# TrondVQ/UncertaintyQuantification-SleepApnea-1DCNN

Measured on AMD Instinct MI355X. Metric: 30s-windows/sec for MCD T=50 & DE M=8 inference at 1/2/4/8 MI355X, higher is better.
Workload: dtype fp32; 1 GPU; global_batch=16384, seq_len=60, parallelism=dp1, mcd_passes=50, de_members=8, bn_mode_mcd=batch

## Files before the change

### uncertaintyquantification_sleepapnea_1dcnn_amd/csrc/x3_layers.hip

```cpp
#include "common.h"
#include "f16x3.h"
#include "x3_api.h"
#include "x3_dense_map.h"

namespace apneauq {
namespace x3 {

constexpr int kStagers = 4;
constexpr int kL = 60, kSR = 64, kHalo = 4;
__host__ __device__ constexpr int row_bytes(int ck) { return 4 * ck + 32; }
__device__ __forceinline__ int sample_prescale(unsigned rmax_bits, const float* amax) {
  return prescale_exp(__builtin_fmaf(amax[0], __uint_as_float(rmax_bits), amax[1]));
}

__host__ __device__ constexpr int lds_rows(int S) { return kHalo + S * kSR + kHalo; }
__host__ __device__ constexpr int buf_bytes(int S, int ck) { return lds_rows(S) * row_bytes(ck); }
__host__ __device__ constexpr int tab_rows(int S, int ks) { return kSR * S + (ks - 1); }
__host__ __device__ constexpr int lds_bytes(int S, int cout, int ck, int ks, bool dense_rows = false) {
  return 2 * (dense_rows ? dense::lds_rows(kSR * S) * row_bytes(ck) : buf_bytes(S, ck)) + 2 * cout * 8 + 2 * S * 4 +
         (dense_rows ? 2 * kSR * S * 4 + 2 * tab_rows(S, ks) * 8 : 0);
}

template <typename T>
__device__ __forceinline__ T gld(const void* p) {
  return *(const __attribute__((address_space(1))) T*)(p);
}

__device__ __forceinline__ int opaque_tid() {
  int t = threadIdx.x;
  asm volatile("" : "+v"(t));
  return t;
}

__device__ __forceinline__ void lds_barrier() {
  __builtin_amdgcn_fence(__ATOMIC_RELEASE, "workgroup", "local");
  __builtin_amdgcn_s_barrier();
  __builtin_amdgcn_fence(__ATOMIC_ACQUIRE, "workgroup", "local");
}

template <int NW, int WPC>
constexpr int waves_per_eu() { return NW * WPC > 8 ? (NW * WPC + 3) / 4 : NW * WPC <= 4 ? 1 : 2; }
constexpr int loaders(int lw) { return lw > 0 ? lw : 0; }
template <int CIN, int COUT, int KS, int S, int WM, int WN, bool LAST, int LW, int CK, int WPC, bool PS, bool DENSE = false>
__global__ __launch_bounds__((WM * WN + loaders(LW)) * 64, (waves_per_eu<WM * WN + loaders(LW), WPC>())) void layer_kernel(
    const LayerArgs A) {
  extern __shared__ __attribute__((aligned(16))) char smem[];
  constexpr int NWM = WM * WN, NW = NWM + loaders(LW), kThreads = NW * 64;
  constexpr int kCK = CK, kRowB = row_bytes(CK), NQ = CK / 32, kQ = CK / 4;
  constexpr int PAD = (KS - 1) / 2, kRows = kSR * S;
  static_assert(!DENSE || (!PS && !LAST), "dense rows: batch-moment blocks 2..5 only");
  constexpr int kS = S, kBufB = DENSE ? dense::lds_rows(kRows) * kRowB : buf_bytes(S, CK);
  constexpr int kValidRows = DENSE ? kRows : S * kL, kUnits = kValidRows * kQ;
  constexpr int SW = LW > 0 ? LW : LW < 0 ? (-LW < NW ? -LW : NW) : (kStagers < NW ? kStagers : NW);
  constexpr int kSBase = LW > 0 ? NWM * 64 : 0;
  constexpr int kST = SW * 64;
  constexpr int kMainU = (kUnits + kST - 1) / kST, kNU = kMainU + (DENSE ? 1 : 0);
  constexpr int kEdgeWaves = (2 * PAD * kQ + 63) / 64;
  static_assert(!DENSE || (kUnits % kST == 0 && kEdgeWaves <= SW), "dense rows: whole staging steps per tile");
  static_assert(kST % kQ == 0 && (CK == 32 || CK == 64), "a staging thread keeps one channel quad");
  constexpr int NCH = CIN / kCK, NCTA = COUT / 16, NCT = NCTA / WN, NRT = 4 * S / WM;
  constexpr int NSTEP = NCH * NQ * KS;
  constexpr int RG = NCT >= 4                        ? 1
                     : (NCT >= 3 && NCT * NRT > 16)    ? 1
                     : NCT == 1                        ? 4
                                                       : 2;
  constexpr bool BDB = NCT * NRT <= 24 && RG < 4;
  static_assert(NRT % RG == 0, "row-tile groups");
  constexpr long long FRAG_STEP = (long long)NCTA * 128;
  static_assert(CIN % kCK == 0 && COUT % 16 == 0, "channel tiling");
  static_assert(NCTA % WN == 0 && (4 * S) % WM == 0, "wave tiling");
  static_assert(NRT % 4 == 0, "whole 64-row sample slots per wave row (epilogue keys, block 6 sums)");
  double* st = reinterpret_cast<double*>(smem + 2 * kBufB);
  float* wsc = reinterpret_cast<float*>(smem + 2 * kBufB + 2 * COUT * 8);
  constexpr int kTabRows = tab_rows(S, KS);
  static_assert(!DENSE || CIN / CK >= 2, "row tables: a tile's tables are written one chunk of the same workgroup ahead");
  unsigned* ektab = reinterpret_cast<unsigned*>(smem + 2 * kBufB + 2 * COUT * 8 + 2 * S * 4);
  uint2* stab = reinterpret_cast<uint2*>(smem + 2 * kBufB + 2 * COUT * 8 + 2 * S * 4 + 2 * kRows * 4);

  const int tid = threadIdx.x, lane = tid & 63;
  const int wave = __builtin_amdgcn_readfirstlane(tid >> 6);
  const int wn = wave % WN, wm = (wave / WN) % WM;
  const int ct0 = wn * NCT, rt0 = wm * NRT;
  const int m = lane & 15, h = lane >> 4;
  APNEAUQ_DASSERT(blockDim.x == kThreads);

  const int wg = xcd_order(blockIdx.x, gridDim.x);
  const int tpg = DENSE ? (int)dense::tiles(A.n_win, kRows) : (A.n_win + S - 1) / S;
  const int total_tiles = tpg * A.groups;
  const int t_begin = (int)((long long)wg * total_tiles / gridDim.x);
  const int t_end = (int)((long long)(wg + 1) * total_tiles / gridDim.x);
  if (t_begin >= t_end) return;
  const int slot = wg % kStatSlots;

  const bool loader = LW > 0 && wave >= NWM;
  const bool stager = LW > 0 ? loader : wave < SW;
  const bool edge_wave = DENSE && wave >= kSBase / 64 && wave - kSBase / 64 < kEdgeWaves;
  auto unit_row = [&](int u, int tid, int& rel) -> bool {
    const int r = tid / kQ;
    if (u < kMainU) {
      rel = r + (kST / kQ) * u;
      return true;
    }
    rel = r < PAD ? r - PAD : kRows - PAD + r;
    return edge_wave && r < 2 * PAD;
  };
  struct Stage {
    f32x4 v[kNU];
    f32x4 a, b;
  };
  Stage s0;
  const bool hash_in = A.thr_in != 0u && !A.sign_in;
  const bool sign_in = A.thr_in != 0u && A.sign_in;
  const bool prescale = PS && A.smax_in != nullptr;
  int key_tile = -1;
  unsigned skeys[kS];
  unsigned skey_tile = 0u;
  static_assert(kS <= 8, "packed per-sample exponents");
  constexpr int kSP = (kS + 3) / 4;
  unsigned sa_pack[kSP];
  struct Geo {
    int g, w0, wf, off, rows_left;
  };
  auto tile_geo = [&](int tile) {
    Geo G;
    G.g = tile / tpg;
    G.w0 = (tile - G.g * tpg) * (DENSE ? kRows : kS);
    G.wf = DENSE ? G.w0 / kL : G.w0, G.off = DENSE ? G.w0 - G.wf * kL : 0;
    const long long left = (long long)(A.n_win - G.wf) * kL - G.off;
    G.rows_left = (int)(left < 1024 ? left : 1024);
    return G;
  };
  const bool mask_out = DENSE && A.sign_out && A.thr_out != 0u;
  auto write_tables = [&](int tile) {
    if constexpr (DENSE) {
      const int tid = opaque_tid() - kSBase;
      const Geo G = tile_geo(tile);
      const unsigned ikey = stream_key(A.seed, A.layer - 1, A.pass_base + G.g);
      const unsigned okey = stream_key(A.seed, A.layer, A.pass_base + G.g);
#pragma unroll
      for (int i0 = 0; i0 < kTabRows; i0 += kST) {
        const int i = i0 + tid, rel = i - PAD;
        if (i < kTabRows) {
          const unsigned d = dense::row_desc(rel, G.off, kRows, PAD, G.rows_left);
          const unsigned win = A.window_offset + G.wf + dense::desc_slot(d);
          const int t = dense::desc_step(d);
          stab[(tile & 1) * kTabRows + i] = uint2{d, hash_in ? dense::mask_word(sample_key(ikey, win), t) : 0u};
          if (mask_out && rel >= 0 && rel < kRows) ektab[(tile & 1) * kRows + rel] = dense::mask_word(sample_key(okey, win), t);
        }
      }
    }
  };
  auto load_chunk = [&](int tile, int c, Stage& R) {
    const int tid = opaque_tid() - kSBase, q = tid % kQ;
    const Geo G = tile_geo(tile);
    const float* af = A.aff_in + (long long)G.g * A.aff_gstride + c * kCK + 4 * q;
    R.a = gld<f32x4>(af);
    R.b = gld<f32x4>(af + CIN);
    if constexpr (DENSE) {
      const long long row0 = (A.in_shared ? 0ll : (long long)G.g * A.n_win * kL) + G.w0;
      const float* in = A.in + row0 * CIN + c * kCK + 4 * q;
#pragma unroll
      for (int u = 0; u < kNU; ++u) {
        int rel;
        bool have = unit_row(u, tid, rel);
        if (u >= kMainU) have = have && dense::staged(G.off + rel, G.off, kRows, PAD);
        R.v[u] = f32x4{-0.f, -0.f, -0.f, -0.f};
        if (have && rel < G.rows_left) R.v[u] = gld<f32x4>(in + rel * CIN);
      }
    } else {
#pragma unroll
      for (int u = 0; u < kNU; ++u) {
        const int ri = tid / kQ + (kST / kQ) * u;
        R.v[u] = f32x4{-0.f, -0.f, -0.f, -0.f};
        if (ri < kValidRows) {
          const int s = ri / kL, t = ri - s * kL, w = G.w0 + s;
          if (w < A.n_win) {
            const long long si = A.in_shared ? w : (long long)G.g * A.n_win + w;
            R.v[u] = gld<f32x4>(A.in + (si * kL + t) * CIN + c * kCK + 4 * q);
          }
        }
      }
    }
  };
  auto store_chunk = [&](int tile, int c, char* buf, const Stage& R) {
    const int tid = opaque_tid() - kSBase, q = tid % kQ;
    const int g = tile / tpg;
    const int w0 = (tile - g * tpg) * (DENSE ? kRows : kS);
    if (DENSE && c == NCH - 1 && tile + 1 < t_end) write_tables(tile + 1);
    if (tile != key_tile) {
      const unsigned skey = stream_key(A.seed, A.layer - 1, A.pass_base + g);
      skey_tile = skey;
      const float* am = A.amax_in + (A.aff_gstride ? 2 * g : 0);
      float ws0 = A.wscale[A.p_gstride ? g : 0];
      if (A.gscale_in != nullptr) ws0 *= A.gscale_in[A.aff_gstride ? g : 0];
#pragma unroll
      for (int i = 0; i < kSP; ++i) sa_pack[i] = 0u;
      if (DENSE && tid == 0) wsc[(tile & 1) * kS] = ws0;
#pragma unroll
      for (int s = 0; s < (DENSE ? 0 : kS); ++s) {
        skeys[s] = sample_key(skey, A.window_offset + w0 + s);
        int sa = 0;
        if (prescale && w0 + s < A.n_win) {
          const long long si = A.in_shared ? w0 + s : (long long)g * A.n_win + w0 + s;
          sa = sample_prescale(A.smax_in[si], am);
          sa_pack[s >> 2] |= ((unsigned)sa & 0xFFu) << (8 * (s & 3));
        }
        if (tid == s) wsc[(tile & 1) * kS + s] = ldexpf(ws0, -sa);
      }
      key_tile = tile;
    }
    const uint2* tab = stab + (tile & 1) * kTabRows + PAD;
#pragma unroll
    for (int u = 0; u < kNU; ++u) {
      int s, lrow;
      bool valid;
      unsigned kt = 0u;
      if constexpr (DENSE) {
        int rel;
        if (!unit_row(u, tid, rel)) continue;
        const uint2 e = tab[rel];
        if (e.x == 0u) continue;
        s = dense::desc_slot(e.x), lrow = dense::desc_lds_row(e.x), valid = dense::desc_valid(e.x), kt = e.y;
      } else {
        const int ri = tid / kQ + (kST / kQ) * u;
        if (ri >= kValidRows) continue;
        s = ri / kL;
        const int t = ri - s * kL;
        lrow = kHalo + s * kSR + t, valid = w0 + s < A.n_win;
        if (hash_in) {
          unsigned k;
          if constexpr (!PS) {
            k = sample_key(skey_tile, A.window_offset + w0 + s);
          } else {
            k = skeys[0];
#pragma unroll
            for (int j = 1; j < kS; ++j) k = s == j ? skeys[j] : k;
          }
          kt = dense::mask_word(k, t);
        }
      }
      const f32x4 v = R.v[u];
      bool keep[4];
      if (hash_in) {
        const unsigned cp = (unsigned)(c * kCK + 4 * q) >> 1;
        const unsigned b01 = mix32(kt ^ cp), b23 = mix32(kt ^ (cp + 1u));
        keep[0] = (b01 & 0xFFFFu) >= A.thr_in;
        keep[1] = (b01 >> 16) >= A.thr_in;
        keep[2] = (b23 & 0xFFFFu) >= A.thr_in;
        keep[3] = (b23 >> 16) >= A.thr_in;
      } else if (sign_in) {
#pragma unroll
        for (int i = 0; i < 4; ++i) keep[i] = !__builtin_signbit(v[i]);
      } else {
#pragma unroll
        for (int i = 0; i < 4; ++i) keep[i] = true;
      }
      int sa = 0;
      if (prescale) {
        unsigned sp = sa_pack[0];
#pragma unroll
        for (int i = 1; i < kSP; ++i) sp = (s >> 2) == i ? sa_pack[i] : sp;
        sa = __builtin_amdgcn_sbfe((int)sp, 8 * (s & 3), 8);
      }
      float a[4];
#pragma unroll
      for (int i = 0; i < 4; ++i) a[i] = (valid && keep[i]) ? ldexpf(__builtin_fmaf(v[i], R.a[i], R.b[i]), sa) : 0.f;
      uint2 hi, lo;
      split2(a[0], a[1], hi.x, lo.x);
      split2(a[2], a[3], hi.y, lo.y);
      char* row = buf + lrow * kRowB + 8 * q;
      *reinterpret_cast<uint2*>(row) = hi;
      *reinterpret_cast<uint2*>(row + 2 * kCK) = lo;
    }
  };

  f32x4 acc[NCT][NRT];
#pragma unroll
  for (int ct = 0; ct < NCT; ++ct)
#pragma unroll
    for (int rt = 0; rt < NRT; ++rt) acc[ct][rt] = f32x4{0.f, 0.f, 0.f, 0.f};
  auto wbase = [&](int tile) -> const gf16x8* {
    const int g = tile / tpg;
    return (const gf16x8*)(A.wfrag) + (long long)g * A.w_gstride + ct0 * 128 + lane;
  };
  f16x8 ah[NCT], al[NCT];
  auto load_a = [&](const gf16x8* p, f16x8 (&xh)[NCT], f16x8 (&xl)[NCT]) {
#pragma unroll
    for (int ct = 0; ct < NCT; ++ct) {
      xh[ct] = p[ct * 128];
      xl[ct] = p[ct * 128 + 64];
    }
  };

  const int bofs = ((rt0 * 16 + m + kHalo - PAD) * kRowB) + 16 * h;

  auto compute_chunk = [&](int c, int off, const char* buf, const gf16x8* wcur, const gf16x8* wnxt, auto&& hook) {
    const char* bp[DENSE ? NRT : 1];
    if constexpr (DENSE) {
#pragma unroll
      for (int rt = 0; rt < NRT; ++rt)
        bp[rt] = buf + bofs + (off + (dense::kSlot - kL) * ((off + (rt0 + rt) * 16 + m) / kL)) * kRowB;
    }
#pragma unroll
    for (int kk = 0; kk < NQ * KS; ++kk) {
      const int q2 = kk / KS, j = kk - q2 * KS;
      const char* bb = buf + bofs + q2 * 64;
      const int s = c * NQ * KS + kk;
      const gf16x8* np = (s + 1 < NSTEP) ? wcur + (long long)(s + 1) * FRAG_STEP : wnxt;
      f16x8 nh[NCT], nl[NCT];
      load_a(np, nh, nl);
      __builtin_amdgcn_sched_barrier(0);
      auto ldb = [&](int rt, f16x8& h_, f16x8& l_) {
        const char* br = DENSE ? bp[rt] + q2 * 64 : bb;
        h_ = *reinterpret_cast<const f16x8*>(br + (rt * 16 + j) * kRowB);
        l_ = *reinterpret_cast<const f16x8*>(br + (rt * 16 + j) * kRowB + 2 * kCK);
      };
      f16x8 bh[RG], bl[RG];
#pragma unroll
      for (int r = 0; r < RG; ++r) ldb(r, bh[r], bl[r]);
#pragma unroll
      for (int rg = 0; rg < NRT; rg += RG) {
        f16x8 bh2[RG], bl2[RG];
#pragma unroll
        for (int r = 0; r < RG; ++r) {
          bh2[r] = bh[r];
          bl2[r] = bl[r];
          if (BDB && rg + RG < NRT) ldb(rg + RG + r, bh2[r], bl2[r]);
          if (!BDB) ldb(rg + r, bh[r], bl[r]);
        }
        __builtin_amdgcn_sched_barrier(0);
#pragma unroll
        for (int r = 0; r < RG; ++r)
#pragma unroll
          for (int ct = 0; ct < NCT; ++ct) acc[ct][rg + r] = mfma(ah[ct], bh[r], acc[ct][rg + r]);
#pragma unroll
        for (int r = 0; r < RG; ++r)
#pragma unroll
          for (int ct = 0; ct < NCT; ++ct) acc[ct][rg + r] = mfma(al[ct], bh[r], acc[ct][rg + r]);
#pragma unroll
        for (int r = 0; r < RG; ++r)
#pragma unroll
          for (int ct = 0; ct < NCT; ++ct) acc[ct][rg + r] = mfma(ah[ct], bl[r], acc[ct][rg + r]);
#pragma unroll
        for (int r = 0; r < RG; ++r) {
          bh[r] = bh2[r];
          bl[r] = bl2[r];
        }
      }
#pragma unroll
      for (int ct = 0; ct < NCT; ++ct) {
        ah[ct] = nh[ct];
        al[ct] = nl[ct];
      }
      __builtin_amdgcn_sched_barrier(0);
      if (kk == (NQ * KS) / 2) hook();
    }
  };

  auto epilogue = [&](int tile) {
    const int lane = opaque_tid() & 63, m = lane & 15, h = lane >> 4;
    const int g = tile / tpg;
    const int w0 = (tile - g * tpg) * (DENSE ? kRows : kS);
    float wsq[NRT / 4];
#pragma unroll
    for (int q = 0; q < NRT / 4; ++q) wsq[q] = wsc[(tile & 1) * kS + (DENSE ? 0 : (rt0 >> 2) + q)];
    const bool track = PS && !LAST && A.smax_out != nullptr;
    float mxs[NRT / 4];
#pragma unroll
    for (int q = 0; q < NRT / 4; ++q) mxs[q] = 0.f;
    const float* bias = A.bias + (long long)g * A.p_gstride;
    const bool drop = (LAST || A.sign_out) && A.thr_out != 0u;
    constexpr int NKEY = DENSE ? 1 : NRT / 4;
    unsigned skeys[NKEY];
    if (!DENSE && drop) {
      const unsigned skey = stream_key(A.seed, A.layer, A.pass_base + g);
#pragma unroll
      for (int q = 0; q < NKEY; ++q) skeys[q] = sample_key(skey, A.window_offset + w0 + (rt0 >> 2) + q);
    }
    const long long left = (long long)A.n_win * kL - w0;
    const int rows_left = DENSE ? (int)(left < kRows ? left : kRows) : 0;
#pragma unroll
    for (int ct = 0; ct < NCT; ++ct) {
      const int co0 = (ct0 + ct) * 16 + 4 * h;
      const f32x4 b4 = gld<f32x4>(bias + co0);
      f32x4 s1 = {0.f, 0.f, 0.f, 0.f}, s2 = s1, k1 = s1, k0 = s1;
      int mo = m;
      if constexpr (DENSE) asm volatile("" : "+v"(mo));
      const int rel0 = rt0 * 16 + mo;
      const unsigned* ek = ektab + (tile & 1) * kRows + rel0;
      float* orow = DENSE ? A.out + (((long long)g * A.n_win * kL + w0 + rel0) * COUT + co0) : nullptr;
#pragma unroll
      for (int rt = 0; rt < NRT; ++rt) {
        int t = 0, w = 0;
        bool valid;
        if constexpr (DENSE) {
          valid = rel0 + rt * 16 < rows_left;
        } else {
          const int s = (rt0 + rt) >> 2;
          t = (((rt0 + rt) & 3) << 4) + m, w = w0 + s, valid = t < kL && w < A.n_win;
        }
        f32x4 r;
#pragma unroll
        for (int e = 0; e < 4; ++e) r[e] = fmaxf(__builtin_fmaf(acc[ct][rt][e], wsq[rt >> 2], b4[e]), 0.f);
        acc[ct][rt] = f32x4{0.f, 0.f, 0.f, 0.f};
        bool keep[4] = {true, true, true, true};
        if (drop) {
          unsigned b01, b23;
          if constexpr (DENSE) {
            const unsigned kt = ek[rt * 16];
            b01 = mix32(kt ^ ((unsigned)co0 >> 1)), b23 = mix32(kt ^ (((unsigned)co0 >> 1) + 1u));
          } else {
            b01 = dropout_bits2(skeys[rt >> 2], t, co0), b23 = dropout_bits2(skeys[rt >> 2], t, co0 + 2);
          }
          keep[0] = (b01 & 0xFFFFu) >= A.thr_out;
          keep[1] = (b01 >> 16) >= A.thr_out;
          keep[2] = (b23 & 0xFFFFu) >= A.thr_out;
          keep[3] = (b23 >> 16) >= A.thr_out;
        }
        if (valid) {
#pragma unroll
          for (int e = 0; e < 4; ++e) {
            s1[e] += r[e];
            s2[e] = __builtin_fmaf(r[e], r[e], s2[e]);
            if (!LAST) mxs[rt >> 2] = fmaxf(mxs[rt >> 2], r[e]);
            if constexpr (LAST) {
              k1[e] += keep[e] ? r[e] : 0.f;
              k0[e] += keep[e] ? 1.f : 0.f;
            }
          }
          if constexpr (!LAST) {
            const long long sample = (long long)g * A.n_win + w;
            f32x4 o = r;
            if (drop) {
#pragma unroll
              for (int e = 0; e < 4; ++e) o[e] = keep[e] ? r[e] : __builtin_copysignf(r[e], -1.f);
            }
            if constexpr (DENSE)
              *reinterpret_cast<f32x4*>(orow + rt * 16 * COUT) = o;
            else
              *reinterpret_cast<f32x4*>(A.out + (sample * kL + t) * COUT + co0) = o;
          }
        }
        if constexpr (LAST) {
          if ((rt & 3) == 3) {
#pragma unroll
            for (int e = 0; e < 4; ++e) {
              k1[e] = group16_sum(k1[e]);
              k0[e] = group16_sum(k0[e]);
            }
            const int wl = w0 + (rt0 + rt) / 4;
            if (m == 0 && wl < A.n_win) {
              float* o = A.out + ((long long)g * A.n_win + wl) * (2 * COUT);
              *reinterpret_cast<f32x4*>(o + co0) = k1;
              *reinterpret_cast<f32x4*>(o + COUT + co0) = k0;
            }
            k1 = f32x4{0.f, 0.f, 0.f, 0.f};
            k0 = k1;
          }
        }
      }
      if (A.stats != nullptr) {
#pragma unroll
        for (int e = 0; e < 4; ++e) {
          const float a = group16_sum(s1[e]), b = group16_sum(s2[e]);
          if (m == 0) {
            atomicAdd(&st[co0 + e], (double)a);
            atomicAdd(&st[COUT + co0 + e], (double)b);
          }
        }
      }
    }
    if (track) {
#pragma unroll
      for (int q = 0; q < NRT / 4; ++q) {
        const float mq = wave_max(mxs[q]);
        const int w = w0 + (rt0 >> 2) + q;
        if (lane == 0 && w < A.n_win) atomicMax(A.smax_out + (long long)g * A.n_win + w, __float_as_uint(mq));
      }
    }
  };

  auto flush_stats = [&](int g) {
    __syncthreads();
    if (A.stats != nullptr) {
      double* dst = A.stats + ((long long)g * kStatSlots + slot) * 2 * COUT;
      for (int i = DENSE ? opaque_tid() : tid; i < 2 * COUT; i += kThreads) {
        atomicAdd(dst + i, st[i]);
        st[i] = 0.0;
      }
    }
    __syncthreads();
  };

  for (int i = tid; i < 2 * kBufB / 16; i += kThreads) reinterpret_cast<f32x4*>(smem)[i] = f32x4{0.f, 0.f, 0.f, 0.f};
  for (int i = tid; i < 2 * COUT; i += kThreads) st[i] = 0.0;
  if (DENSE && stager) write_tables(t_begin);
  __syncthreads();
  const int total = (t_end - t_begin) * NCH;
  auto chunk_tile = [&](int it) { return t_begin + it / NCH; };
  auto tile_off = [&](int tile) { return DENSE ? (int)((long long)(tile % tpg) * kRows % kL) : 0; };
  int g_cur = t_begin / tpg;
  if constexpr (LW > 0) {
    if (loader) {
      if (stager) {
        load_chunk(t_begin, 0, s0);
        store_chunk(t_begin, 0, smem, s0);
      }
      lds_barrier();
      if (stager && total > 1) load_chunk(chunk_tile(1), 1 % NCH, s0);
#pragma unroll 1
      for (int it = 0; it < total; ++it) {
        const int tile = chunk_tile(it), c = it - (tile - t_begin) * NCH;
        if (c == 0) {
          const int g = tile / tpg;
          if (g != g_cur) {
            flush_stats(g_cur);
            g_cur = g;
          }
        }
        if (stager && it + 1 < total) store_chunk(chunk_tile(it + 1), (it + 1) % NCH, smem + ((it + 1) & 1) * kBufB, s0);
        lds_barrier();
        if (stager && it + 2 < total) load_chunk(chunk_tile(it + 2), (it + 2) % NCH, s0);
      }
      flush_stats(g_cur);
      return;
    }
    lds_barrier();
    load_a(wbase(t_begin), ah, al);
#pragma unroll 1
    for (int it = 0; it < total; ++it) {
      const int tile = chunk_tile(it), c = it - (tile - t_begin) * NCH;
      if (c == 0) {
        const int g = tile / tpg;
        if (g != g_cur) {
          flush_stats(g_cur);
          g_cur = g;
        }
      }
      const gf16x8* wcur = wbase(tile);
      const gf16x8* wnxt = wbase(tile + 1 < t_end ? tile + 1 : tile);
      compute_chunk(c, tile_off(tile), smem + (it & 1) * kBufB, wcur, wnxt, []() {});
      if (c == NCH - 1) epilogue(tile);
      lds_barrier();
    }
    flush_stats(g_cur);
    return;
  }
  if (stager) {
    load_chunk(t_begin, 0, s0);
    store_chunk(t_begin, 0, smem, s0);
  }
  lds_barrier();
  if (stager && total > 1) load_chunk(chunk_tile(1), 1 % NCH, s0);
  load_a(wbase(t_begin), ah, al);
#pragma unroll 1
  for (int it = 0; it < total; ++it) {
    const int tile = chunk_tile(it), c = it - (tile - t_begin) * NCH;
    if (c == 0) {
      const int g = tile / tpg;
      if (g != g_cur) {
        flush_stats(g_cur);
        g_cur = g;
      }
    }
    const gf16x8* wcur = wbase(tile);
    const gf16x8* wnxt = wbase(tile + 1 < t_end ? tile + 1 : tile);
    char* buf = smem + (it & 1) * kBufB;
    char* nbuf = smem + ((it + 1) & 1) * kBufB;
    compute_chunk(c, tile_off(tile), buf, wcur, wnxt, [&]() {
      if (stager && it + 1 < total) store_chunk(chunk_tile(it + 1), (it + 1) % NCH, nbuf, s0);
    });
    if (c == NCH - 1) epilogue(tile);
    lds_barrier();
    if (stager && it + 2 < total) load_chunk(chunk_tile(it + 2), (it + 2) % NCH, s0);
  }
  flush_stats(g_cur);
}

__global__ __launch_bounds__(256) void l1_kernel(const L1Args A) {
  __shared__ float xs[kL1Win][kL + 6][4];
  __shared__ float red[2][2][128];
  __shared__ unsigned wmax[kL1Win];
  const int g = blockIdx.x / A.blocks_per_group;
  const int w0 = (blockIdx.x - g * A.blocks_per_group) * kL1Win;
  const int tid = threadIdx.x, c = tid & 127, half = tid >> 7;
  for (int i = tid; i < kL1Win * (kL + 6) * 4; i += 256) {
    const int s = i / ((kL + 6) * 4), r = (i / 4) % (kL + 6), ci = i & 3;
    const int t = r - 3, w = w0 + s;
    xs[s][r][ci] = (t >= 0 && t < kL && w < A.n_win) ? A.x[((long long)w * kL + t) * 4 + ci] : 0.f;
  }
  float wr[7][4];
#pragma unroll
  for (int j = 0; j < 7; ++j)
#pragma unroll
    for (int ci = 0; ci < 4; ++ci) wr[j][ci] = A.w[(((long long)g * 7 + j) * 4 + ci) * 128 + c];
  const float bc = A.b[g * 128 + c];
  if (tid < kL1Win) wmax[tid] = 0u;
  __syncthreads();
  float s1 = 0.f, s2 = 0.f;
  for (int s = 0; s < kL1Win; ++s) {
    const int w = w0 + s;
    if (w >= A.n_win) break;
    float* o = A.out + (((long long)g * A.n_win + w) * kL) * 128 + c;
    float mx = 0.f;
    for (int t = half * 30; t < half * 30 + 30; ++t) {
      float v = bc;
#pragma unroll
      for (int j = 0; j < 7; ++j)
#pragma unroll
        for (int ci = 0; ci < 4; ++ci) v = __builtin_fmaf(xs[s][t + j][ci], wr[j][ci], v);
      v = fmaxf(v, 0.f);
      o[t * 128] = v;
      s1 += v;
      s2 = __builtin_fmaf(v, v, s2);
      mx = fmaxf(mx, v);
    }
    if (A.smax != nullptr) {
      mx = wave_max(mx);
      if ((tid & 63) == 0) atomicMax(&wmax[s], __float_as_uint(mx));
    }
  }
  if (A.stats != nullptr || A.smax != nullptr) {
    red[half][0][c] = s1;
    red[half][1][c] = s2;
    __syncthreads();
    if (A.stats != nullptr && tid < 128) {
      double* dst = A.stats + ((long long)g * kStatSlots + (blockIdx.x % kStatSlots)) * 2 * 128;
      atomicAdd(dst + c, (double)red[0][0][c] + (double)red[1][0][c]);
      atomicAdd(dst + 128 + c, (double)red[0][1][c] + (double)red[1][1][c]);
    }
    if (A.smax != nullptr && tid < kL1Win && w0 + tid < A.n_win) A.smax[(long long)g * A.n_win + w0 + tid] = wmax[tid];
  }
}

__device__ __forceinline__ void aff_moments(const AffArgs& A, int g, int c, float& mean, float& var) {
  const double* p = A.stats + (long long)g * kStatSlots * 2 * A.C + c;
  double a = 0.0, b = 0.0;
#pragma unroll
  for (int s = 0; s < kStatSlots; ++s) {
    a += p[s * 2 * A.C];
    b += p[s * 2 * A.C + A.C];
  }
  const double mu = a * A.inv_count;
  mean = (float)mu;
  var = (float)fmax(b * A.inv_count - mu * mu, 0.0);
}

__global__ __launch_bounds__(256) void aff_kernel(const AffArgs A) {
  __shared__ float red[2][4];
  const int tid = threadIdx.x;
  if ((int)blockIdx.x == A.groups) {
    for (int c = tid; c < A.C; c += 256)
      for (int g = 0; g < A.groups; ++g) {
        const long long po = (long long)g * A.p_gstride + c;
        float mean, var;
        aff_moments(A, g, c, mean, var);
        for (int r = 0; r < A.repeat; ++r) {
          A.mmean[po] = A.mmean[po] * A.momentum + mean * (1.f - A.momentum);
          A.mvar[po] = A.mvar[po] * A.momentum + var * (1.f - A.momentum);
        }
      }
    return;
  }
  {
    const int g = blockIdx.x;
    float ms = 0.f, mt = 0.f;
    for (int c = tid; c < A.C; c += 256) {
      const long long po = (long long)g * A.p_gstride + c;
      float mean, var;
      if (A.stats != nullptr && !A.running) {
        aff_moments(A, g, c, mean, var);
      } else {
        mean = A.mmean[po];
        var = A.mvar[po];
      }
      const float sc = A.gamma[po] / sqrtf(var + A.eps);
      const float s_ = sc * A.dsc, t_ = (A.beta[po] - mean * sc) * A.dsc;
      A.aff[((long long)g * 2) * A.C + c] = s_;
      A.aff[((long long)g * 2 + 1) * A.C + c] = t_;
      if (A.gscale != nullptr) {
        const double* p = A.stats + (long long)g * kStatSlots * 2 * A.C + A.C + c;
        double q = 0.0;
        for (int s = 0; s < kStatSlots; ++s) q += p[s * 2 * A.C];
        ms = fmaxf(ms, __builtin_fmaf(fabsf(s_), (float)sqrt(fmax(q, 0.0)) * 1.0001f, fabsf(t_)));
      } else {
        ms = fmaxf(ms, fabsf(s_));
        mt = fmaxf(mt, fabsf(t_));
      }
    }
    if (A.gscale != nullptr) {
      ms = wave_max(ms);
      if ((tid & 63) == 0) red[0][tid >> 6] = ms;
      __syncthreads();
      const float bnd = fmaxf(fmaxf(red[0][0], red[0][1]), fmaxf(red[0][2], red[0][3]));
      int e = 0;
      if (bnd > 0.f && bnd < INFINITY) frexpf(bnd, &e);
      const int sa = min(100, max(-100, 14 - e));
      for (int c = tid; c < A.C; c += 256) {
        float* af = A.aff + (long long)g * 2 * A.C + c;
        af[0] = ldexpf(af[0], sa);
        af[A.C] = ldexpf(af[A.C], sa);
      }
      if (tid == 0) A.gscale[g] = ldexpf(1.f, -sa);
      return;
    }
    if (A.amax == nullptr) return;
    ms = wave_max(ms);
    mt = wave_max(mt);
    if ((tid & 63) == 0) {
      red[0][tid >> 6] = ms;
      red[1][tid >> 6] = mt;
    }
    __syncthreads();
    if (tid == 0) {
      A.amax[2 * g] = fmaxf(fmaxf(red[0][0], red[0][1]), fmaxf(red[0][2], red[0][3]));
      A.amax[2 * g + 1] = fmaxf(fmaxf(red[1][0], red[1][1]), fmaxf(red[1][2], red[1][3]));
    }
  }
}

__global__ __launch_bounds__(256) void head_kernel(const HeadArgs A) {
  const int lane = threadIdx.x & 63;
  const long long sidx = (long long)blockIdx.x * 4 + (threadIdx.x >> 6);
  if (sidx >= A.samples) return;
  const int g = (int)(sidx / A.n_win);
  const float* s = A.sums + sidx * 2 * A.C;
  const float* af = A.aff + (long long)g * A.aff_gstride;
  const float* dw = A.dw + (long long)g * A.p_gstride;
  float v = 0.f;
  for (int c = lane; c < A.C; c += 64) v += dw[c] * __builtin_fmaf(af[c], s[c], af[A.C + c] * s[A.C + c]);
  v = wave_sum(v);
  if (lane == 0) {
    const float logit = v * (1.0f / kL) + A.db[A.p_gstride ? g : 0];
    A.out[sidx] = A.out_logits ? logit : 1.0f / (1.0f + expf(-logit));
  }
}

template <int CIN, int COUT, int KS, int S, int WM, int WN, bool LAST, int LW, int CK, int WPC, bool PS, bool DENSE = false>
hipError_t launch_layer(const LayerArgs& A, int grid, hipStream_t stream) {
  constexpr int lds = lds_bytes(S, COUT, CK, KS, DENSE);
  static_assert(WPC * lds <= 160 * 1024, "LDS of the workgroups sharing a CU");
  auto k = layer_kernel<CIN, COUT, KS, S, WM, WN, LAST, LW, CK, WPC, PS, DENSE>;
  static bool attr = false;
  if (!attr) {
    hipError_t e = hipFuncSetAttribute(reinterpret_cast<const void*>(k), hipFuncAttributeMaxDynamicSharedMemorySize, lds);
    if (e != hipSuccess) return e;
    attr = true;
  }
  hipLaunchKernelGGL(k, dim3(grid), dim3((WM * WN + loaders(LW)) * 64), lds, stream, A);
  return hipGetLastError();
}

template <bool HAVE, int CIN, int COUT, int KS, int S, int WM, int WN, int LW, int CK, int WPC>
hipError_t launch_dense(const LayerArgs& A, int grid, hipStream_t stream) {
  if constexpr (HAVE) {
    return launch_layer<CIN, COUT, KS, S, WM, WN, false, (LW > 0 ? LW : -(WM * WN)), CK, WPC, false, true>(A, grid, stream);
  } else {
    return hipErrorInvalidValue;
  }
}

}

#ifdef APNEAUQ_X3_TABLE
#include APNEAUQ_X3_TABLE
#else
#define APNEAUQ_X3_LAYERS(X)                           \
  X(1, 128, 192, 5, 4, 2, 4, false, -8, 0, 32, 1, true) \
  X(2, 192, 224, 3, 2, 1, 7, false, 4, 4, 64, 1, true)  \
  X(3, 224, 96, 7, 4, 2, 2, false, 4, 4, 32, 1, true)   \
  X(4, 96, 256, 9, 2, 1, 8, false, 4, 4, 32, 1, true)   \
  X(5, 256, 96, 9, 4, 2, 2, true, 4, 4, 64, 1, false)
#endif

int x3_lds_bytes(int layer) {
#define APNEAUQ_X3_LDS(L, CI, CO, K, S, WM, WN, LAST, LW, LWB, CK, WPC, DENSE) \
  if (layer == L) return x3::lds_bytes(S, CO, CK, K);
  APNEAUQ_X3_LAYERS(APNEAUQ_X3_LDS)
#undef APNEAUQ_X3_LDS
  return 0;
}

int x3_tile_samples(int layer) {
#define APNEAUQ_X3_TS(L, CI, CO, K, S, WM, WN, LAST, LW, LWB, CK, WPC, DENSE) \
  if (layer == L) return S;
  APNEAUQ_X3_LAYERS(APNEAUQ_X3_TS)
#undef APNEAUQ_X3_TS
  return 0;
}

bool x3_has_dense(int layer) {
#define APNEAUQ_X3_HD(L, CI, CO, K, S, WM, WN, LAST, LW, LWB, CK, WPC, DENSE) \
  if (layer == L) return DENSE && !LAST;
  APNEAUQ_X3_LAYERS(APNEAUQ_X3_HD)
#undef APNEAUQ_X3_HD
  return false;
}

int x3_wg_per_cu(int layer) {
#define APNEAUQ_X3_WPC(L, CI, CO, K, S, WM, WN, LAST, LW, LWB, CK, WPC, DENSE) \
  if (layer == L) return WPC;
  APNEAUQ_X3_LAYERS(APNEAUQ_X3_WPC)
#undef APNEAUQ_X3_WPC
  return 1;
}

hipError_t x3_launch_layer(int layer, const x3::LayerArgs& A, int grid, bool dense_rows, hipStream_t stream) {
  using namespace x3;
  const bool ps = A.smax_in != nullptr || A.smax_out != nullptr;
#define APNEAUQ_X3_LAUNCH(L, CI, CO, K, S, WM, WN, LAST, LW, LWB, CK, WPC, DENSE)                                  \
  if (layer == L) {                                                                                       \
    if (dense_rows)                                                                                       \
      return ps ? hipErrorInvalidValue                                                                    \
                : launch_dense<DENSE && !LAST, CI, CO, K, S, WM, WN, LWB, CK, WPC>(A, grid, stream);       \
    return ps ? launch_layer<CI, CO, K, S, WM, WN, LAST, LW, CK, WPC, true>(A, grid, stream)               \
              : launch_layer<CI, CO, K, S, WM, WN, LAST, LWB, CK, WPC, false>(A, grid, stream);            \
  }
  APNEAUQ_X3_LAYERS(APNEAUQ_X3_LAUNCH)
#undef APNEAUQ_X3_LAUNCH
  return hipErrorInvalidValue;
}

hipError_t x3_launch_l1(const x3::L1Args& A, hipStream_t stream) {
  const int grid = A.groups * A.blocks_per_group;
  if (grid <= 0) return hipSuccess;
  hipLaunchKernelGGL(x3::l1_kernel, dim3(grid), dim3(256), 0, stream, A);
  return hipGetLastError();
}

hipError_t x3_launch_aff(const x3::AffArgs& A, hipStream_t stream) {
  const int blocks = A.groups + (A.stats != nullptr && A.update ? 1 : 0);
  hipLaunchKernelGGL(x3::aff_kernel, dim3(blocks), dim3(256), 0, stream, A);
  return hipGetLastError();
}

hipError_t x3_launch_head(const x3::HeadArgs& A, hipStream_t stream) {
  if (A.samples <= 0) return hipSuccess;
  hipLaunchKernelGGL(x3::head_kernel, dim3((A.samples + 3) / 4), dim3(256), 0, stream, A);
  return hipGetLastError();
}

}
```

Before: 67790 windows/s.

## Precompute dropout mask bits on loader waves into LDS table; hoist bias loads

For the dense 96->256 k9 layer with dedicated loader waves, the loader threads now compute the output dropout keep-bits during the chunk iterations ahead of a tile's last one. They store these as a packed per-row/per-column-tile LDS table. The epilogue then applies sign flips with bit ops instead of hashing per element, moving hash work off the compute waves' critical path. Bias loads are also hoisted ahead of the epilogue loop for dense layers. This costs extra LDS per workgroup, which may reduce occupancy, and adds loader work between barriers.

```diff
diff --git a/uncertaintyquantification_sleepapnea_1dcnn_amd/csrc/x3_layers.hip b/uncertaintyquantification_sleepapnea_1dcnn_amd/csrc/x3_layers.hip
--- a/uncertaintyquantification_sleepapnea_1dcnn_amd/csrc/x3_layers.hip
+++ b/uncertaintyquantification_sleepapnea_1dcnn_amd/csrc/x3_layers.hip
@@ -16,9 +16,13 @@
 __host__ __device__ constexpr int lds_rows(int S) { return kHalo + S * kSR + kHalo; }
 __host__ __device__ constexpr int buf_bytes(int S, int ck) { return lds_rows(S) * row_bytes(ck); }
 __host__ __device__ constexpr int tab_rows(int S, int ks) { return kSR * S + (ks - 1); }
-__host__ __device__ constexpr int lds_bytes(int S, int cout, int ck, int ks, bool dense_rows = false) {
+__host__ __device__ constexpr int mask_tab_bytes(int S, int cout) { return kSR * S * (cout / 16) * 2; }
+__host__ __device__ constexpr bool mask_tab_layer(int cin, int cout, int ks, int lw, bool dense_rows) {
+  return dense_rows && lw > 0 && cin == 96 && cout == 256 && ks == 9;
+}
+__host__ __device__ constexpr int lds_bytes(int S, int cout, int ck, int ks, bool dense_rows = false, bool mask_tab = false) {
   return 2 * (dense_rows ? dense::lds_rows(kSR * S) * row_bytes(ck) : buf_bytes(S, ck)) + 2 * cout * 8 + 2 * S * 4 +
-         (dense_rows ? 2 * kSR * S * 4 + 2 * tab_rows(S, ks) * 8 : 0);
+         (dense_rows ? 2 * kSR * S * 4 + 2 * tab_rows(S, ks) * 8 : 0) + (dense_rows && mask_tab ? mask_tab_bytes(S, cout) : 0);
 }
 
 template <typename T>
@@ -76,6 +80,13 @@
   static_assert(!DENSE || CIN / CK >= 2, "row tables: a tile's tables are written one chunk of the same workgroup ahead");
   unsigned* ektab = reinterpret_cast<unsigned*>(smem + 2 * kBufB + 2 * COUT * 8 + 2 * S * 4);
   uint2* stab = reinterpret_cast<uint2*>(smem + 2 * kBufB + 2 * COUT * 8 + 2 * S * 4 + 2 * kRows * 4);
+  constexpr bool kMaskTab = mask_tab_layer(CIN, COUT, KS, LW, DENSE);
+  constexpr bool kBiasHoist = DENSE;
+  constexpr int kMtRowW = COUT / 16, kMtT = kMaskTab ? kST / kRows : 1, kMtW = kMtRowW / kMtT;
+  constexpr int kMtPhase = (kMtW + (NCH > 1 ? NCH - 2 : 0)) / (NCH > 1 ? NCH - 1 : 1);
+  static_assert(!kMaskTab || NCH >= 2, "mask table: written in the chunk iterations ahead of the tile's last");
+  static_assert(!kMaskTab || (kST % kRows == 0 && kMtRowW % kMtT == 0), "mask table: whole words per loader thread");
+  unsigned short* mtab = reinterpret_cast<unsigned short*>(smem + 2 * kBufB + 2 * COUT * 8 + 2 * S * 4 + 2 * kRows * 4 + 2 * kTabRows * 8);
 
   const int tid = threadIdx.x, lane = tid & 63;
   const int wave = __builtin_amdgcn_readfirstlane(tid >> 6);
@@ -146,6 +157,27 @@
           const int t = dense::desc_step(d);
           stab[(tile & 1) * kTabRows + i] = uint2{d, hash_in ? dense::mask_word(sample_key(ikey, win), t) : 0u};
           if (mask_out && rel >= 0 && rel < kRows) ektab[(tile & 1) * kRows + rel] = dense::mask_word(sample_key(okey, win), t);
+        }
+      }
+    }
+  };
+  auto draw_mask = [&](int tile, int c) {
+    if constexpr (kMaskTab) {
+      const int tid = opaque_tid() - kSBase, row = tid / kMtT, w0 = (tid % kMtT) * kMtW;
+      const unsigned kt = ektab[(tile & 1) * kRows + row];
+      unsigned short* dst = mtab + row * kMtRowW + w0;
+#pragma unroll
+      for (int j = 0; j < kMtPhase; ++j) {
+        const int i = c * kMtPhase + j;
+        if (i < kMtW) {
+          const unsigned cp = (unsigned)(w0 + i) * 8u;
+          unsigned bits = 0u;
+#pragma unroll
+          for (int p = 0; p < 8; ++p) {
+            const unsigned b = mix32(kt ^ (cp + p));
+            bits |= ((b & 0xFFFFu) >= A.thr_out ? 1u : 0u) << (2 * p) | ((b >> 16) >= A.thr_out ? 1u : 0u) << (2 * p + 1);
+          }
+          dst[i] = (unsigned short)bits;
         }
       }
     }
@@ -379,15 +411,27 @@
     }
     const long long left = (long long)A.n_win * kL - w0;
     const int rows_left = DENSE ? (int)(left < kRows ? left : kRows) : 0;
+    f32x4 bq[kBiasHoist ? NCT : 1];
+    if constexpr (kBiasHoist) {
+#pragma unroll
+      for (int ct = 0; ct < NCT; ++ct) bq[ct] = gld<f32x4>(bias + (ct0 + ct) * 16 + 4 * h);
+#pragma unroll
+      for (int ct = 0; ct < NCT; ++ct) asm volatile("" : "+v"(bq[ct]));
+    }
 #pragma unroll
     for (int ct = 0; ct < NCT; ++ct) {
       const int co0 = (ct0 + ct) * 16 + 4 * h;
-      const f32x4 b4 = gld<f32x4>(bias + co0);
+      f32x4 b4;
+      if constexpr (kBiasHoist)
+        b4 = bq[ct];
+      else
+        b4 = gld<f32x4>(bias + co0);
       f32x4 s1 = {0.f, 0.f, 0.f, 0.f}, s2 = s1, k1 = s1, k0 = s1;
       int mo = m;
       if constexpr (DENSE) asm volatile("" : "+v"(mo));
       const int rel0 = rt0 * 16 + mo;
       const unsigned* ek = ektab + (tile & 1) * kRows + rel0;
+      const unsigned short* mt = mtab + rel0 * kMtRowW + (ct0 + ct);
       float* orow = DENSE ? A.out + (((long long)g * A.n_win * kL + w0 + rel0) * COUT + co0) : nullptr;
 #pragma unroll
       for (int rt = 0; rt < NRT; ++rt) {
@@ -404,7 +448,10 @@
         for (int e = 0; e < 4; ++e) r[e] = fmaxf(__builtin_fmaf(acc[ct][rt][e], wsq[rt >> 2], b4[e]), 0.f);
         acc[ct][rt] = f32x4{0.f, 0.f, 0.f, 0.f};
         bool keep[4] = {true, true, true, true};
-        if (drop) {
+        unsigned sgn = 0u;
+        if constexpr (kMaskTab) {
+          if (drop) sgn = ~((unsigned)mt[rt * 16 * kMtRowW] >> (4 * h));
+        } else if (drop) {
           unsigned b01, b23;
           if constexpr (DENSE) {
             const unsigned kt = ek[rt * 16];
@@ -431,7 +478,10 @@
           if constexpr (!LAST) {
             const long long sample = (long long)g * A.n_win + w;
             f32x4 o = r;
-            if (drop) {
+            if constexpr (kMaskTab) {
+#pragma unroll
+              for (int e = 0; e < 4; ++e) o[e] = __uint_as_float(__float_as_uint(r[e]) | ((sgn << (31 - e)) & 0x80000000u));
+            } else if (drop) {
 #pragma unroll
               for (int e = 0; e < 4; ++e) o[e] = keep[e] ? r[e] : __builtin_copysignf(r[e], -1.f);
             }
@@ -519,6 +569,7 @@
           }
         }
         if (stager && it + 1 < total) store_chunk(chunk_tile(it + 1), (it + 1) % NCH, smem + ((it + 1) & 1) * kBufB, s0);
+        if (kMaskTab && stager && mask_out && c < NCH - 1) draw_mask(tile, c);
         lds_barrier();
         if (stager && it + 2 < total) load_chunk(chunk_tile(it + 2), (it + 2) % NCH, s0);
       }
@@ -738,7 +789,7 @@
 
 template <int CIN, int COUT, int KS, int S, int WM, int WN, bool LAST, int LW, int CK, int WPC, bool PS, bool DENSE = false>
 hipError_t launch_layer(const LayerArgs& A, int grid, hipStream_t stream) {
-  constexpr int lds = lds_bytes(S, COUT, CK, KS, DENSE);
+  constexpr int lds = lds_bytes(S, COUT, CK, KS, DENSE, mask_tab_layer(CIN, COUT, KS, LW, DENSE));
   static_assert(WPC * lds <= 160 * 1024, "LDS of the workgroups sharing a CU");
   auto k = layer_kernel<CIN, COUT, KS, S, WM, WN, LAST, LW, CK, WPC, PS, DENSE>;
   static bool attr = false;
```

Measured after the change: 68780 windows/s, median of 6. +1.5%, better.
